# dbry/audio-resampler

Hardware: AMD Instinct MI355X
Metric: Msamples/s (out) 44.1k->48k preset -4, 8ch float32 (higher is better)
Workload: dtype i8 x 4 digits (32-bit fixed point of the f32 samples and the fp64-blended filter rows, exact i32 accumulation, one float rounding per output)

## Files before the change

audio_resampler_amd/csrc/fir_matrix_i8.hip:

```cpp
#include "fir_matrix_stream.hip.h"
#include <atomic>
#include <cstdlib>

#if !ART_WIDE

namespace {

typedef int i32x4 __attribute__ ((ext_vector_type (4)));
typedef int i32x16 __attribute__ ((ext_vector_type (16)));

constexpr int I8_KC = 32;
constexpr int I8_PITCH = 48;
constexpr int I8_COLS = 128;
constexpr int I8_MAX_PPW = 64;
constexpr int i8_ppw (int cols, int cg) { return cols / cg > I8_MAX_PPW ? I8_MAX_PPW : cols / cg; }
constexpr float I8_SCALE = 1073741824.0f;
constexpr float I8_LIMIT = 1.98f;

struct I8Geom {
    int tr;
    int cols;
    int tiles;
    int ktot;
    int g;
// ... 425 lines not shown

        for (int ch = 0; ch < nchunks; ++ch, ++qn) {
            const unsigned char *Ab = &As_ [0] [0] [0] + (qn & 1) * (int) sizeof (As_ [0]) + aoff;
            const unsigned char *Bb = &Bs_ [0] [0] [0] + (qn & 1) * (int) sizeof (Bs_ [0]) + boff;
            i32x4 av [4], bv [4];
#pragma unroll
            for (int pn = 0; pn < 4; ++pn) {
                av [pn] = *reinterpret_cast<const i32x4 *> (Ab + pn * (32 * I8_PITCH));
                bv [pn] = *reinterpret_cast<const i32x4 *> (Bb + pn * (I8_COLS * I8_PITCH));
            }
            __builtin_amdgcn_sched_group_barrier (0x100, 8, 0);
            __syncthreads ();
#define I8_PART 4
#include "fir_i8_tile32.inc"
        }
#define I8_PART 5
#include "fir_i8_tile32.inc"
    }
}

typedef __attribute__ ((address_space (3))) void *lds_ptr_t;

template <int CG, bool PASS>
__global__ __launch_bounds__ (2 * MF_THREADS) __attribute__ ((amdgpu_waves_per_eu (4, 4)))
void fir_i8_dma_kernel (ArtFirArgs a, MfmaGeom g, I8Geom q, int wgs_per_xcd)
{
    static_assert (CG >= 4 && I8_COLS % CG == 0, "16-byte vectors of 4 channels");
    constexpr int THREADS = 2 * MF_THREADS;
    constexpr int PPW = I8_COLS / CG;
    constexpr int NBUF = 3, A_BUF = 4096, B_BUF = 16384;
    __shared__ __attribute__ ((aligned (16))) unsigned char As_ [NBUF * A_BUF];
    __shared__ __attribute__ ((aligned (16))) unsigned char Bs_ [NBUF * B_BUF];

    const int tid = threadIdx.x, lane = tid & 63, wave = tid >> 6;
    const bool loader = wave >= 4;

#define I8_PART 1
#include "fir_i8_tile32.inc"
    const int total = my_tiles * nchunks;

    if (loader) {
        constexpr int VPF = CG / 4;
        constexpr unsigned int A_STEP = 4096u, B_STEP = (I8_KC / 4) * CG * 4u;
        const int lw = wave - 4;
        const int kb = 2 * lw + (lane >> 5), colquad = lane & 31, m = colquad / VPF, cv = colquad - m * VPF;
        const unsigned int boff = (unsigned int)((m * q.gq4 + kb) * CG + cv * 4) * 4u;
        const unsigned int a_off = (unsigned int)(lw * 1024 + lane * 16);
        constexpr int NB = 1;
        const int bper [NB] = { m * q.g };
        unsigned int bdel [NB] = { 0u };
        const __attribute__ ((address_space (4))) int *tile_w0 = (const __attribute__ ((address_space (4))) int *) g.tile_w0;

#define I8_PART 2
#include "fir_i8_tile32.inc"
        auto issue = [&] (int buf) -> bool {
            if (!f_live) return false;
            const unsigned int sa = (unsigned int) f_chunk * A_STEP, sb = min ((unsigned int) f_chunk * B_STEP, fb_bytes);
            const __amdgpu_buffer_rsrc_t ra_ = make_rsrc (fa_base + sa, fa_bytes - sa), rb_ = make_rsrc (fb_base + sb, fb_bytes - sb);
            __builtin_amdgcn_raw_ptr_buffer_load_lds (ra_, (lds_ptr_t)(As_ + buf * A_BUF + lw * 1024), 16, (int) a_off, 0, 0, 0);
#pragma unroll
            for (int pn = 0; pn < 4; ++pn)
                __builtin_amdgcn_raw_ptr_buffer_load_lds (rb_, (lds_ptr_t)(Bs_ + buf * B_BUF + pn * 4096 + lw * 1024), 16, (int)(boff + bdel [0]), (int)((unsigned int) pn * q.eb_plane_bytes), 0, 0);
            if (++f_chunk == nchunks) { f_chunk = 0; open_tile (); }
            return true;
        };

        open_tile ();
        bool all = true;
#pragma unroll
        for (int b = 0; b < NBUF - 1; ++b) all = issue (b) && all;
        if (all) { if constexpr (NBUF == 3) asm volatile ("s_waitcnt vmcnt(5)" ::: "memory"); else asm volatile ("s_waitcnt vmcnt(10)" ::: "memory"); }
        else asm volatile ("s_waitcnt vmcnt(0)" ::: "memory");
        __builtin_amdgcn_s_barrier ();
        int fill = NBUF - 1;
        for (int c = 0; c < total; ++c) {
            const bool more = issue (fill);
            fill = fill == NBUF - 1 ? 0 : fill + 1;
            if (more) { if constexpr (NBUF == 3) asm volatile ("s_waitcnt vmcnt(5)" ::: "memory"); else asm volatile ("s_waitcnt vmcnt(10)" ::: "memory"); }
            else asm volatile ("s_waitcnt vmcnt(0)" ::: "memory");
            __builtin_amdgcn_s_barrier ();
        }
        return;
    }

    {
        const unsigned int hw_id = __builtin_amdgcn_s_getreg ((4 - 1) << 11 | 16 << 6 | 4);
        if (hw_id & 1u) __builtin_amdgcn_s_setprio (3); else __builtin_amdgcn_s_setprio (0);
    }
    const int col = wave * 32 + (lane & 31);
    constexpr bool col_live = true;
    const int jl = col / CG, c = col - jl * CG;
    const unsigned char *Ab0 = As_ + (lane & 31) * 16 + (lane >> 5) * 512;
    const unsigned char *Bb0 = Bs_ + (lane >> 5) * 2048 + col * 4;
    const unsigned int out_off = (unsigned int)((jl * q.g * g.P + 4 * (lane >> 5)) * CG + c) * 4u;

    __builtin_amdgcn_s_barrier ();
    asm volatile ("" ::: "memory");
    int qb = 0;
    for (int within = rank; within < tiles_per_xcd; within += wgs_per_xcd) {
        int st, j0;
        if (!tile_at (within, st, j0)) continue;
#define I8_PART 3
#include "fir_i8_tile32.inc"

        for (int ch = 0; ch < nchunks; ++ch) {
            const unsigned char *Ab = Ab0 + qb * A_BUF, *Bb = Bb0 + qb * B_BUF;
            qb = qb == NBUF - 1 ? 0 : qb + 1;
            i32x4 av [4], bv [4];
#pragma unroll
            for (int pn = 0; pn < 4; ++pn) {
                av [pn] = *reinterpret_cast<const i32x4 *> (Ab + pn * 1024);
#pragma unroll
                for (int i = 0; i < 4; ++i) bv [pn] [i] = *reinterpret_cast<const int *> (Bb + pn * 4096 + i * 512);
            }
            __builtin_amdgcn_sched_group_barrier (0x100, 12, 0);
            asm volatile ("s_waitcnt lgkmcnt(0)" ::: "memory");
            __builtin_amdgcn_s_barrier ();
            asm volatile ("" ::: "memory");
#define I8_PART 4
#include "fir_i8_tile32.inc"
        }
#define I8_PART 5
#include "fir_i8_tile32.inc"
    }
}


constexpr int SL_COLS = 256, SL_THREADS = 512;
constexpr int SL_A_IMG = 8192, SL_B_IMG = 32768, SL_IMG = SL_A_IMG + SL_B_IMG, SL_BUF = 2 * SL_IMG;
constexpr int SL_WGS = 32;
constexpr int SL_MAX_SK = 64;
constexpr size_t SL_PART_BYTES = (size_t) 8 * 16 * 64 * 16;

struct I8Slab {
    int wgs_per_xcd;
    int live [8];
    unsigned char *parts;
    unsigned int *arrivals;
};


template <int CG, bool PASS>
__global__ __launch_bounds__ (SL_THREADS) __attribute__ ((amdgpu_waves_per_eu (2, 2)))
void fir_i8_slab_kernel (ArtFirArgs a, MfmaGeom g, I8Geom q, I8Slab sl)
{
    static_assert (CG >= 4 && SL_COLS % CG == 0 && SL_COLS / CG <= I8_MAX_PPW, "16-byte vectors of 4 channels");
    constexpr int THREADS = SL_THREADS;
    constexpr int PPW = SL_COLS / CG;
    __shared__ __attribute__ ((aligned (16))) unsigned char smem_ [2 * SL_BUF];

    const int tid = threadIdx.x, lane = tid & 63;
    const int wave = __builtin_amdgcn_readfirstlane (tid >> 6);

    if (a.roll_dst) {
        for (int e = (int) blockIdx.x * THREADS + tid; e < a.H * a.C; e += (int) gridDim.x * THREADS)
            matrix_roll (a.roll_dst, a.hist, a.in, a.in_frames, a.H, a.C, a.roll_appended, e);
    }
    const int W = sl.wgs_per_xcd;
    if (*q.flag == q.epoch) {
        constexpr int MF_PPW = MF_COLS / CG > MF_MAX_PPW ? MF_MAX_PPW : MF_COLS / CG;
        (void) MF_PPW;
        stand_by_tiles<CG, PASS> (a, g, W, *reinterpret_cast<float (*) [2] [32 * MF_LD]> (&smem_ [0]), *reinterpret_cast<float (*) [2] [MF_COLS * MF_LD]> (&smem_ [SL_BUF]));
        return;
    }

    const int xcd = blockIdx.x & 7, rank = blockIdx.x >> 3;
    const int nsub = q.ktot / I8_KC, nch = (nsub + 1) >> 1;
    const int L = sl.live [xcd];
    if (L <= 0) return;
    int D, S;
    {
        const int R = L / W, rem = L - R * W;
        D = rem ? (R > 0 ? R - 1 : 0) : R;
        S = L - D * W;
    }
    const int Ct = S * nch, Weff = S ? (W < Ct ? W : Ct) : 1;
    const int lo = S && rank < Weff ? (rank * Ct) / Weff : 0, hi = S && rank < Weff ? ((rank + 1) * Ct) / Weff : 0;
    const int t_first = lo / nch, t_last = hi > lo ? (hi - 1) / nch : t_first - 1;
    const int nseg = D + (t_last - t_first + 1);
    if (nseg == 0) return;
    auto segment = [&] (int k, int &within, int &c0, int &c1) {
        if (k < D) { within = rank + k * W; c0 = 0; c1 = nch; }
        else {
            const int t = t_first + (k - D);
            within = D * W + t;
            c0 = lo - t * nch; if (c0 < 0) c0 = 0;
            c1 = hi - t * nch; if (c1 > nch) c1 = nch;
        }
    };
    const int g_mask = q.g - 1, g_log2 = q.g >> 1;
    auto tile_of = [&] (int within, int &st, int &j0) {
        st = within % q.tiles;
        const int t2 = within / q.tiles, jr = t2 & g_mask, sg = xcd * q.sg_per_xcd + (t2 >> g_log2);
        j0 = ((sg * PPW) << g_log2) + jr;
    };

    constexpr int VPF = CG / 4;
    constexpr unsigned int A_STEP = 8192u, B_STEP = (I8_KC / 4) * CG * 4u;
    const int kb = 2 * (wave & 3) + (lane >> 5), colquad = (wave >> 2) * 32 + (lane & 31), m = colquad / VPF, cv = colquad - m * VPF;
    const unsigned int boff = (unsigned int)((m * q.gq4 + kb) * CG + cv * 4) * 4u;
    const unsigned int a_off = (unsigned int)(wave * 1024 + lane * 16);
    const unsigned int x_total = 4u * q.eb_plane_bytes;
    const unsigned int eb_hop = x_total - (unsigned int) q.eb_step * (unsigned int)(CG * 4);
    const int plane_step = __builtin_amdgcn_readfirstlane ((int) q.eb_plane_bytes);
    const __attribute__ ((address_space (4))) int *tile_w0 = (const __attribute__ ((address_space (4))) int *) g.tile_w0;

    int f_seg = -1, f_ch = 0, f_c1 = 0;
    unsigned long long f_live [2] = { 0ull, 0ull };
    __amdgpu_buffer_rsrc_t f_ra = make_rsrc (nullptr, 0u), f_rb = f_ra;
    unsigned int f_va = 0u, f_vb = 0u;
    auto open_segment = [&] () {
        int within, st, j0, c0;
        ++f_seg;
        segment (f_seg, within, c0, f_c1);
        tile_of (within, st, j0);
        const int la = max (tile_w0 [3 * (2 * st)] + g.w_shift + j0 * g.Q + g.head_pad, 0);
        const int eb = j0 / q.eb_periods;
        unsigned int skip = (unsigned int) max ((la >> 2) - q.b0 - eb * q.eb_step, 0) * (unsigned int)(CG * 4);
        if (skip > q.eb_plane_bytes) skip = q.eb_plane_bytes;
        const size_t from = (size_t) eb * x_total + skip;
        f_rb = make_rsrc (q.x_planes + from, (unsigned int) min (q.x_bytes - from, (size_t) 0xfffffff0u));
        const unsigned int fa_bytes = (unsigned int) nsub * A_STEP;
        f_ra = make_rsrc (q.a_planes + (size_t)(st * q.g + ((j0 + q.jr_rot) & g_mask)) * fa_bytes, fa_bytes);
        {
            const __attribute__ ((address_space (4))) unsigned long long *tm = (const __attribute__ ((address_space (4))) unsigned long long *) q.tile_masks + (st * q.g + ((j0 + q.jr_rot) & g_mask)) * 2;
            f_live [0] = tm [0] | tm [1];
            f_live [1] = tm [q.tiles * q.g * 2] | tm [q.tiles * q.g * 2 + 1];
        }
        f_ch = c0;
        f_va = a_off + (unsigned int)(2 * c0) * A_STEP;
        f_vb = boff + (unsigned int)((j0 + m * q.g) / q.eb_periods - eb) * eb_hop + (unsigned int)(2 * c0) * B_STEP;
    };
    int total = D * nch + (hi - lo), issued = 0;
    unsigned int d_va = 0u, d_vb = 0u;
    int d_skip [2] = { 0, 0 };
    int d_skip3 [2] = { 0, 0 };
    auto next_chunk = [&] () {
        if (issued < total) {
            if (f_seg < 0 || f_ch == f_c1) open_segment ();
            d_va = f_va; d_vb = f_vb;
#pragma unroll
            for (int im = 0; im < 2; ++im) {
                d_skip [im] = (wave >> 1) < 2 && !((f_live [wave >> 1] >> (2 * f_ch + im)) & 1ull) ? 0x7ffffff0 : 0;
                d_skip3 [im] = !(((f_live [0] | f_live [1]) >> (2 * f_ch + im)) & 1ull) ? 0x7ffffff0 : 0;
            }
            f_va += 2 * A_STEP; f_vb += 2 * B_STEP;
            ++f_ch; ++issued;
        }
        else { f_ra = make_rsrc (nullptr, 0u); f_rb = f_ra; }
    };
    auto piece = [&] (int buf, int idx) {
        const int im = idx / 5, pc = idx % 5;
        unsigned char *img = smem_ + buf * SL_BUF + im * SL_IMG;
        if (pc == 0) __builtin_amdgcn_raw_ptr_buffer_load_lds (f_ra, (lds_ptr_t)(img + wave * 1024), 16, (int)(d_va + (unsigned int) im * A_STEP), d_skip [im], 0, 0);
        else __builtin_amdgcn_raw_ptr_buffer_load_lds (f_rb, (lds_ptr_t)(img + SL_A_IMG + (pc - 1) * 8192 + wave * 1024), 16, (int)(d_vb + (unsigned int) im * B_STEP), pc == 4 ? (d_skip3 [im] ? d_skip3 [im] : 3 * plane_step) : (pc - 1) * plane_step, 0, 0);
    };

    if (wave & 4) __builtin_amdgcn_s_setprio (2); else __builtin_amdgcn_s_setprio (0);
    const int col = wave * 32 + (lane & 31);
    const int jl = col / CG, c = col - jl * CG;
    const unsigned char *Ab0 = smem_ + (lane >> 5) * 1024 + (lane & 31) * 16;
    const unsigned char *Bb0 = smem_ + SL_A_IMG + (wave >> 2) * 4096 + (lane >> 5) * 2048 + (col & 127) * 4;

    next_chunk ();
#pragma unroll
    for (int idx = 0; idx < 10; ++idx) piece (0, idx);
    asm volatile ("s_waitcnt vmcnt(0)" ::: "memory");
    __builtin_amdgcn_s_barrier ();
    asm volatile ("" ::: "memory");
    next_chunk ();
#pragma unroll
    for (int idx = 0; idx < 5; ++idx) piece (1, idx);
    int cur = 0;

    for (int k = 0; k < nseg; ++k) {
        int within, c0, c1, st, j0;
        segment (k, within, c0, c1);
        tile_of (within, st, j0);
        i32x16 acc [2] [5];
#pragma unroll
        for (int h = 0; h < 2; ++h)
#pragma unroll
            for (int s = 0; s < 5; ++s)
#pragma unroll
                for (int r = 0; r < 16; ++r) acc [h] [s] [r] = 0;
        unsigned long long top [2], sec [2];
        {
            const __attribute__ ((address_space (4))) unsigned long long *tm = (const __attribute__ ((address_space (4))) unsigned long long *) q.tile_masks + (st * q.g + ((j0 + q.jr_rot) & g_mask)) * 2;
            top [0] = tm [0]; top [1] = tm [1];
            sec [0] = tm [q.tiles * q.g * 2]; sec [1] = tm [q.tiles * q.g * 2 + 1];
        }
        int shift_v = q.shifts [((j0 + jl * q.g) / q.eb_periods) * CG + c];

        i32x4 av [2] [4], bv [4];
        auto read_image = [&] (int im, int sub) {
            const unsigned char *Ab = Ab0 + cur * SL_BUF + im * SL_IMG, *Bb = Bb0 + cur * SL_BUF + im * SL_IMG;
            const bool l0 = ((top [0] | top [1]) >> sub) & 1ull, l1 = ((sec [0] | sec [1]) >> sub) & 1ull;
            if (l0 | l1) {
                av [0] [1] = *reinterpret_cast<const i32x4 *> (Ab + 2048);
                av [1] [1] = *reinterpret_cast<const i32x4 *> (Ab + 2048 + 512);
#pragma unroll
                for (int i = 0; i < 4; ++i) bv [3] [i] = *reinterpret_cast<const int *> (Bb + 3 * 8192 + i * 512);
                if (l0) {
                    av [0] [0] = *reinterpret_cast<const i32x4 *> (Ab);
                    av [1] [0] = *reinterpret_cast<const i32x4 *> (Ab + 512);
                }
            }
#pragma unroll
            for (int pn = 2; pn < 4; ++pn) {
                av [0] [pn] = *reinterpret_cast<const i32x4 *> (Ab + pn * 2048);
                av [1] [pn] = *reinterpret_cast<const i32x4 *> (Ab + pn * 2048 + 512);
            }
#pragma unroll
            for (int pn = 0; pn < 3; ++pn)
#pragma unroll
                for (int i = 0; i < 4; ++i) bv [pn] [i] = *reinterpret_cast<const int *> (Bb + pn * 8192 + i * 512);
        };
        auto products = [&] (int sub, int to, int first) {
#pragma unroll
            for (int h = 0; h < 2; ++h) {
                int n = 0;
#pragma unroll
                for (int i = 2; i < 4; ++i)
#pragma unroll
                    for (int j = 0; j < 4; ++j)
                        if (i + j <= 4) {
                            acc [h] [i + j] = __builtin_amdgcn_mfma_i32_32x32x32_i8 (av [h] [i], bv [j], acc [h] [i + j], 0, 0, 0);
                            ++n;
                            if (h == 0 && n == 2) piece (to, first);
                            if (h == 0 && n == 4) piece (to, first + 1);
                            if (h == 1 && n == 1) piece (to, first + 2);
                            if (h == 1 && n == 3) piece (to, first + 3);
                            if (h == 1 && n == 5) piece (to, first + 4);
                        }
                if (h == 0) {
                    __builtin_amdgcn_sched_group_barrier (0x008, 2, 0); __builtin_amdgcn_sched_group_barrier (0x020, 1, 0);
                    __builtin_amdgcn_sched_group_barrier (0x008, 2, 0); __builtin_amdgcn_sched_group_barrier (0x020, 1, 0);
                    __builtin_amdgcn_sched_group_barrier (0x008, 1, 0);
                }
                else {
                    __builtin_amdgcn_sched_group_barrier (0x008, 1, 0); __builtin_amdgcn_sched_group_barrier (0x020, 1, 0);
                    __builtin_amdgcn_sched_group_barrier (0x008, 2, 0); __builtin_amdgcn_sched_group_barrier (0x020, 1, 0);
                    __builtin_amdgcn_sched_group_barrier (0x008, 2, 0); __builtin_amdgcn_sched_group_barrier (0x020, 1, 0);
                }
                if ((sec [h] >> sub) & 1ull) {
#pragma unroll
                    for (int j = 0; j < 4; ++j) acc [h] [1 + j] = __builtin_amdgcn_mfma_i32_32x32x32_i8 (av [h] [1], bv [j], acc [h] [1 + j], 0, 0, 0);
                }
                if ((top [h] >> sub) & 1ull) {
#pragma unroll
                    for (int j = 0; j < 4; ++j) acc [h] [j] = __builtin_amdgcn_mfma_i32_32x32x32_i8 (av [h] [0], bv [j], acc [h] [j], 0, 0, 0);
                }
            }
        };

        for (int ch = c0; ch < c1; ++ch) {
            read_image (0, 2 * ch);
            __builtin_amdgcn_sched_group_barrier (0x100, 16, 0);
            products (2 * ch, cur ^ 1, 5);
            const bool two = 2 * ch + 1 < nsub;
            if (two) read_image (1, 2 * ch + 1);
            asm volatile ("s_waitcnt lgkmcnt(0)" ::: "memory");
            asm volatile ("s_waitcnt vmcnt(0)" ::: "memory");
            if (ch == c0) asm volatile ("" : "+v" (shift_v));
            __builtin_amdgcn_s_barrier ();
            asm volatile ("" ::: "memory");
            next_chunk ();
            if (two) products (2 * ch + 1, cur, 0);
            else {
#pragma unroll
                for (int idx = 0; idx < 5; ++idx) piece (cur, idx);
            }
            asm volatile ("" ::: "memory");
            cur ^= 1;
        }

        long long tot [2] [16];
#pragma unroll
        for (int h = 0; h < 2; ++h)
#pragma unroll
            for (int r = 0; r < 16; ++r) tot [h] [r] = i8_total (acc [h] [0] [r], acc [h] [1] [r], acc [h] [2] [r], acc [h] [3] [r], acc [h] [4] [r]);
        if (c0 != 0 || c1 != nch) {
            constexpr int COHERENT = 1 | 16;
            const int t = within - D * W;
            auto owner_of = [&] (int chunk) {
                int r = (int)(((long long) chunk * Weff) / Ct);
                while (r + 1 < Weff && ((r + 1) * Ct) / Weff <= chunk) ++r;
                return r;
            };
            const int r_first = owner_of (t * nch), r_last = owner_of ((t + 1) * nch - 1);
            const unsigned int wave_bytes = 16u * 64u * 16u;
            unsigned int *count = sl.arrivals + ((size_t)(xcd * SL_MAX_SK + t) * 8 + wave);
            unsigned int before = 0u;
            bool look = k == nseg - 1 && k != D;
            if (look) {
                if (lane == 0) before = __hip_atomic_load (count, __ATOMIC_RELAXED, __HIP_MEMORY_SCOPE_AGENT);
                before = (unsigned int) __builtin_amdgcn_readfirstlane ((int) before);
                look = before == (unsigned int)(r_last - r_first);
            }
            if (!look) {
                const int which = k == D ? 0 : 1;
                const __amdgpu_buffer_rsrc_t rs_part = make_rsrc (sl.parts + ((size_t)((xcd * W + rank) * 2 + which) * 8 + wave) * wave_bytes, wave_bytes);
#pragma unroll
                for (int r = 0; r < 16; ++r) {
                    u32x4 v;
                    const unsigned long long x0 = (unsigned long long) tot [0] [r], x1 = (unsigned long long) tot [1] [r];
                    v.x = (unsigned int) x0; v.y = (unsigned int)(x0 >> 32); v.z = (unsigned int) x1; v.w = (unsigned int)(x1 >> 32);
                    __builtin_amdgcn_raw_buffer_store_b128 (v, rs_part, (r * 64 + lane) * 16, 0, COHERENT);
                }
                asm volatile ("s_waitcnt vmcnt(0)" ::: "memory");
                if (lane == 0) before = __hip_atomic_fetch_add (count, 1u, __ATOMIC_RELAXED, __HIP_MEMORY_SCOPE_AGENT);
                before = (unsigned int) __builtin_amdgcn_readfirstlane ((int) before);
            }
            if (before != (unsigned int)(r_last - r_first)) continue;
            if (lane == 0) __hip_atomic_store (count, 0u, __ATOMIC_RELAXED, __HIP_MEMORY_SCOPE_AGENT);
            for (int rr = r_first; rr <= r_last; ++rr) {
                if (rr == rank) continue;
                const int which = (rr * Ct) / Weff / nch == t ? 0 : 1;
                const __amdgpu_buffer_rsrc_t rs_part = make_rsrc (sl.parts + ((size_t)((xcd * W + rr) * 2 + which) * 8 + wave) * wave_bytes, wave_bytes);
                u32x4 v [16];
#pragma unroll
                for (int r = 0; r < 16; ++r) v [r] = __builtin_amdgcn_raw_buffer_load_b128 (rs_part, (r * 64 + lane) * 16, 0, COHERENT);
#pragma unroll
                for (int r = 0; r < 16; ++r) {
                    tot [0] [r] += (long long)((unsigned long long) v [r].x | (unsigned long long) v [r].y << 32);
                    tot [1] [r] += (long long)((unsigned long long) v [r].z | (unsigned long long) v [r].w << 32);
                }
            }
        }
        const int out_exp = -14 - shift_v;
        const unsigned int n_tile = a.n_begin + (unsigned int) j0 * g.P + (unsigned int)(st * 64);
        const int rows_valid = min (64, g.P - st * 64);
        const size_t left = (size_t)(a.n_end - n_tile) * CG * 4;
        const __amdgpu_buffer_rsrc_t rs_out = make_rsrc (a.out + (size_t) n_tile * CG, left > 0xffffff00ull ? 0xffffff00u : (unsigned int) left);
        float y [2] [16];
#pragma unroll
        for (int h = 0; h < 2; ++h) {
            const unsigned int pass_rows = PASS && 2 * st + h < g.slot_tiles ? (unsigned int) tile_w0 [3 * (2 * st + h) + 1] : 0u;
#pragma unroll
            for (int r = 0; r < 16; ++r) {
                y [h] [r] = i8_round (tot [h] [r], out_exp);
                if constexpr (PASS) {
                    const int i = h * 32 + (r & 3) + 8 * (r >> 2) + 4 * (lane >> 5);
                    if ((pass_rows >> (i & 31)) & 1u)
                        y [h] [r] = load_frame (a, INT_MIN, g.canon_ip [st * 64 + i] + g.w_shift + g.canon_fi [st * 64 + i] / a.F + (j0 + jl * q.g) * g.Q, c);
                }
            }
        }
        {
            int lane_e = lane;
            asm volatile ("" : "+v" (lane_e));
            const int qm = lane_e & 3;
            const int lo = a.n_skip != 0 && j0 == 0 && wave == 0 ? a.n_skip - st * 64 : 0;
            const int col_e = wave * 32 + (lane_e & 31), jl_e = col_e / CG, c_e = col_e - jl_e * CG;
            const unsigned int q_off = (unsigned int)((((jl_e << g_log2) * g.P) + 4 * (lane_e >> 5) + qm) * CG + (c_e & ~3)) * 4u;
#pragma unroll
            for (int h = 0; h < 2; ++h)
#pragma unroll
                for (int rb = 0; rb < 4; ++rb) {
                    unsigned int t [4];
#pragma unroll
                    for (int u = 0; u < 4; ++u) t [u] = __float_as_uint (y [h] [4 * rb + u]);
#pragma unroll
                    for (int pr = 0; pr < 4; pr += 2) {
                        const unsigned int send = (qm & 1) ? t [pr] : t [pr + 1];
                        const unsigned int recv = (unsigned int) __builtin_amdgcn_mov_dpp ((int) send, 0xB1, 0xf, 0xf, true);
                        if (qm & 1) t [pr] = recv; else t [pr + 1] = recv;
                    }
#pragma unroll
                    for (int pr = 0; pr < 2; ++pr) {
                        const unsigned int send = (qm & 2) ? t [pr] : t [pr + 2];
                        const unsigned int recv = (unsigned int) __builtin_amdgcn_mov_dpp ((int) send, 0x4E, 0xf, 0xf, true);
                        if (qm & 2) t [pr] = recv; else t [pr + 2] = recv;
                    }
                    u32x4 v; v.x = t [0]; v.y = t [1]; v.z = t [2]; v.w = t [3];
                    const int i_const = h * 32 + 8 * rb;
                    const int i = i_const + 4 * (lane >> 5) + qm;
                    const unsigned int off = i < rows_valid && (i >= lo || (lane & 31) >= CG) ? q_off + (unsigned int)(i_const * CG) * 4u : 0xfffffff0u;
                    __builtin_amdgcn_raw_buffer_store_b128 (v, rs_out, (int) off, 0, 0);
                }
        }
    }
    asm volatile ("s_waitcnt vmcnt(0)" ::: "memory");
}


}

bool artfir_i8_slab_enabled ()
{
    static const bool on = [] { const char *e = getenv ("ARTAMD_I8_SLAB"); return !(e && *e == '0'); } ();
    return on;
}
static int i8_slab_min_tiles ()
{
    static const int v = [] { const char *e = getenv ("ARTAMD_I8_SLAB_MIN"); return e && *e ? atoi (e) : 24; } ();
    return v;
}

static size_t i8_layout (const ArtFirArgs *a, const MfmaGeom &g, int cgt, I8Geom &q, char *base, unsigned int outputs = 0)
{
    if (!cgt || g.tile_rows != 32 || (g.ktot % I8_KC)) return 0;
    const unsigned int total = outputs ? outputs + (unsigned int) g.P : a->n_end - a->n_begin, periods = (total + g.P - 1) / g.P;
    q.g = (g.Q % 4 == 0) ? 1 : (g.Q % 2 == 0) ? 2 : 4;
    q.tr = 32; q.cols = I8_COLS; q.rows_cached = 0; q.jr_rot = 0; q.rows_table = 0; q.tb_base = 0.0; q.tb_lin = q.tb_w = 0; q.tb_n0 = 0u;
    if (artfir_i8_slab_enabled () && cgt >= 4) {
        const int ppw64 = i8_ppw (SL_COLS, cgt);
        const int sgs = (int)((periods + (unsigned int)(q.g * ppw64) - 1) / (unsigned int)(q.g * ppw64));
        const int per_xcd = ((sgs + 7) / 8) * q.g * ((g.P + 63) / 64);
        if (per_xcd >= i8_slab_min_tiles ()) { q.tr = 64; q.cols = SL_COLS; }
    }
    for (;;) {
        const int shift_max = (int)((q.tr - 1.0) * g.Q / g.P) + 2;
        q.ktot = ((a->T + shift_max + 3 + I8_KC - 1) / I8_KC) * I8_KC;
        if (q.tr == 64 && (q.ktot / I8_KC < 4 || q.ktot / I8_KC > 64)) { q.tr = 32; q.cols = I8_COLS; continue; }
        break;
    }
    q.tiles = (g.P + q.tr - 1) / q.tr;
    const int ppw = i8_ppw (q.cols, cgt);
    q.gq4 = q.g * g.Q / 4;
    q.super_groups = (int)((periods + (unsigned int)(q.g * ppw) - 1) / (unsigned int)(q.g * ppw));
    q.sg_per_xcd = (q.super_groups + 7) / 8;
    if (q.ktot / I8_KC > 64) return 0;
    {
        const int unit = 16 * q.g * g.Q;
        const int k = (9408 + unit / 2) / unit;
        q.eb_periods = 16 * q.g * (k > 1 ? k : 1);
    }
    q.eb_step = q.eb_periods * g.Q / 4;
    const int over_blocks = (g.Q + 2 + q.ktot + 3 + 3) / 4 + 2;
    q.eb_blocks = q.eb_step + over_blocks;
    q.ebs = (int)((periods + (unsigned int) q.eb_periods - 1) / (unsigned int) q.eb_periods);
    q.cgrp = a->C < 8 ? a->C : 8;
    q.slice_blocks = I8_STAGE_K * I8_STAGE_THREADS / q.cgrp;
    q.slices = (q.eb_blocks + q.slice_blocks - 1) / q.slice_blocks;
    q.eb_plane_bytes = (unsigned int) q.eb_blocks * (unsigned int) a->C * 4u;
    q.x_bytes = (size_t) q.ebs * 4 * q.eb_plane_bytes;
    q.b0 = 0;
    const size_t a_bytes = (size_t) q.tiles * q.g * (q.ktot / I8_KC) * (size_t)(q.tr * 128);
    const size_t masks = 2 * ((size_t) q.tiles * q.g * q.tr * 8 + (size_t) q.tiles * q.g * (q.tr / 32) * 8), shifts = (size_t) q.ebs * a->C * 4;
    const size_t teams = (size_t) q.ebs * q.slices * a->C * 4;
    const size_t head = (ART_I8_HEAD_BYTES + masks + teams + shifts + 255) & ~(size_t) 255;
    q.flag = (int *) base; q.epoch = 0;
    q.a_masks = (unsigned long long *)(base + ART_I8_HEAD_BYTES);
    q.mask_words = q.tiles * q.g * q.tr;
    q.tile_masks = q.a_masks + 2 * (size_t) q.mask_words;
    q.peaks = (unsigned int *)(base + ART_I8_HEAD_BYTES + masks);
    q.shifts = (int *)(base + ART_I8_HEAD_BYTES + masks + teams);
    q.a_planes = (unsigned char *) base + head;
    q.x_planes_w = (unsigned int *)(base + head + a_bytes); q.x_planes = (const unsigned char *) q.x_planes_w;
    q.parts = q.tr == 64 ? (unsigned char *) base + ((head + a_bytes + q.x_bytes + 255) & ~(size_t) 255) : nullptr;
    return q.tr == 64 ? ((head + a_bytes + q.x_bytes + 255) & ~(size_t) 255) + (size_t) 8 * SL_WGS * 2 * SL_PART_BYTES : head + a_bytes + q.x_bytes;
}

size_t artfir_i8_bytes (const ArtFirArgs *a, const MfmaGeom &g, int cgt, unsigned int outputs)
{
    I8Geom q;
    return i8_layout (a, g, cgt, q, nullptr, outputs ? outputs : 1u);
}

namespace {

struct RowsSetPtrs {
    unsigned long long *a_masks, *tile_masks; unsigned char *a_planes;
    float *eff; double *canon_frac; int *canon_ip, *canon_fi, *tile_w0;
};
static size_t rows_set_layout (const MfmaGeom &g, const I8Geom &q, char *base, RowsSetPtrs *out)
{
    size_t off = 0;
    auto take = [&] (size_t bytes) { const size_t at = off; off = (off + bytes + 255) & ~(size_t) 255; return at; };
    const size_t rows32 = (size_t) g.slot_tiles * 32;
    const size_t o_masks = take (2 * (size_t) q.tiles * q.g * q.tr * 8), o_tm = take (2 * (size_t) q.tiles * q.g * (q.tr / 32) * 8);
    const size_t o_planes = take ((size_t) q.tiles * q.g * (q.ktot / I8_KC) * (size_t)(q.tr * 128));
    const size_t o_eff = take (rows32 * g.ktot * sizeof (float)), o_frac = take (rows32 * sizeof (double));
    const size_t o_ip = take (rows32 * sizeof (int)), o_fi = take (rows32 * sizeof (int)), o_w0 = take ((size_t) 3 * g.slot_tiles * sizeof (int));
    if (out && base) {
        out->a_masks = (unsigned long long *)(base + o_masks); out->tile_masks = (unsigned long long *)(base + o_tm); out->a_planes = (unsigned char *)(base + o_planes);
        out->eff = (float *)(base + o_eff); out->canon_frac = (double *)(base + o_frac); out->canon_ip = (int *)(base + o_ip); out->canon_fi = (int *)(base + o_fi);
        out->tile_w0 = (int *)(base + o_w0);
    }
    return off;
}

}

extern "C" {
size_t arthip_fir_rows_cache_bytes (void) { return sizeof (ArtRowsCache); }
void arthip_fir_rows_cache_reset (void *cache)
{
    ArtRowsCache *rc = (ArtRowsCache *) cache;
    if (rc) { for (int k = 0; k < 4; ++k) rc->valid [k] = 0; rc->f_valid = 0; }
}
void arthip_fir_rows_cache_free (void *cache)
{
    ArtRowsCache *rc = (ArtRowsCache *) cache;
    if (rc) {
        free (rc->c_ph); free (rc->c_ip); free (rc->c_fi); rc->c_ph = nullptr; rc->c_ip = rc->c_fi = nullptr; rc->cap = 0; rc->canon_valid = 0;
    }
}
}

size_t artfir_i8_rows_bytes (const ArtFirArgs *a, const MfmaGeom &g, int cgt, unsigned int outputs)
{
    I8Geom q;
    if (!i8_layout (a, g, cgt, q, nullptr, outputs ? outputs : 1u)) return 0;
    return (size_t)(4 / q.g) * (rows_set_layout (g, q, nullptr, nullptr) + 4096);
}

namespace {

typedef void (*I8TileKernel) (ArtFirArgs, MfmaGeom, I8Geom, int);
typedef void (*I8SlabKernel) (ArtFirArgs, MfmaGeom, I8Geom, I8Slab);
#define I8_PICK(KERNEL, CGT) (pass ? KERNEL<CGT, true> : KERNEL<CGT, false>)
I8TileKernel i8_tile_kernel (int cgt, bool pass)
{
    switch (cgt) {
        case 32: return I8_PICK (fir_i8_dma_kernel, 32);
        case 16: return I8_PICK (fir_i8_dma_kernel, 16);
        case 8: return I8_PICK (fir_i8_dma_kernel, 8);
        case 4: return I8_PICK (fir_i8_dma_kernel, 4);
        case 2: return I8_PICK (fir_i8_stream_kernel, 2);
        default: return I8_PICK (fir_i8_stream_kernel, 1);
    }
}
I8SlabKernel i8_slab_kernel (int cgt, bool pass)
{
    switch (cgt) {
        case 32: return I8_PICK (fir_i8_slab_kernel, 32);
        case 16: return I8_PICK (fir_i8_slab_kernel, 16);
        case 8: return I8_PICK (fir_i8_slab_kernel, 8);
        default: return I8_PICK (fir_i8_slab_kernel, 4);
    }
}
#undef I8_PICK
// ... 130 lines not shown
```

Before: 84050.

## Prefetch first chunk before roll and defer split-tile fixup to overlap waiting

Result: no change. 83220 (-1.0%).

```diff
diff --git a/audio_resampler_amd/csrc/fir_matrix_i8.hip b/audio_resampler_amd/csrc/fir_matrix_i8.hip
--- a/audio_resampler_amd/csrc/fir_matrix_i8.hip
+++ b/audio_resampler_amd/csrc/fir_matrix_i8.hip
@@ -601,22 +601,10 @@
     const int tid = threadIdx.x, lane = tid & 63;
     const int wave = __builtin_amdgcn_readfirstlane (tid >> 6);
 
-    if (a.roll_dst) {
-        for (int e = (int) blockIdx.x * THREADS + tid; e < a.H * a.C; e += (int) gridDim.x * THREADS)
-            matrix_roll (a.roll_dst, a.hist, a.in, a.in_frames, a.H, a.C, a.roll_appended, e);
-    }
     const int W = sl.wgs_per_xcd;
-    if (*q.flag == q.epoch) {
-        constexpr int MF_PPW = MF_COLS / CG > MF_MAX_PPW ? MF_MAX_PPW : MF_COLS / CG;
-        (void) MF_PPW;
-        stand_by_tiles<CG, PASS> (a, g, W, *reinterpret_cast<float (*) [2] [32 * MF_LD]> (&smem_ [0]), *reinterpret_cast<float (*) [2] [MF_COLS * MF_LD]> (&smem_ [SL_BUF]));
-        return;
-    }
-
     const int xcd = blockIdx.x & 7, rank = blockIdx.x >> 3;
     const int nsub = q.ktot / I8_KC, nch = (nsub + 1) >> 1;
-    const int L = sl.live [xcd];
-    if (L <= 0) return;
+    const int L = sl.live [xcd] > 0 ? sl.live [xcd] : 0;
     int D, S;
     {
         const int R = L / W, rem = L - R * W;
@@ -627,7 +615,6 @@
     const int lo = S && rank < Weff ? (rank * Ct) / Weff : 0, hi = S && rank < Weff ? ((rank + 1) * Ct) / Weff : 0;
     const int t_first = lo / nch, t_last = hi > lo ? (hi - 1) / nch : t_first - 1;
     const int nseg = D + (t_last - t_first + 1);
-    if (nseg == 0) return;
     auto segment = [&] (int k, int &within, int &c0, int &c1) {
         if (k < D) { within = rank + k * W; c0 = 0; c1 = nch; }
         else {
@@ -705,15 +692,31 @@
         else __builtin_amdgcn_raw_ptr_buffer_load_lds (f_rb, (lds_ptr_t)(img + SL_A_IMG + (pc - 1) * 8192 + wave * 1024), 16, (int)(d_vb + (unsigned int) im * B_STEP), pc == 4 ? (d_skip3 [im] ? d_skip3 [im] : 3 * plane_step) : (pc - 1) * plane_step, 0, 0);
     };
 
+    if (nseg != 0) {
+        next_chunk ();
+#pragma unroll
+        for (int idx = 0; idx < 10; ++idx) piece (0, idx);
+    }
+    if (a.roll_dst) {
+        for (int e = (int) blockIdx.x * THREADS + tid; e < a.H * a.C; e += (int) gridDim.x * THREADS)
+            matrix_roll (a.roll_dst, a.hist, a.in, a.in_frames, a.H, a.C, a.roll_appended, e);
+    }
+    if (*q.flag == q.epoch) {
+        constexpr int MF_PPW = MF_COLS / CG > MF_MAX_PPW ? MF_MAX_PPW : MF_COLS / CG;
+        (void) MF_PPW;
+        asm volatile ("s_waitcnt vmcnt(0)" ::: "memory");
+        __syncthreads ();
+        stand_by_tiles<CG, PASS> (a, g, W, *reinterpret_cast<float (*) [2] [32 * MF_LD]> (&smem_ [0]), *reinterpret_cast<float (*) [2] [MF_COLS * MF_LD]> (&smem_ [SL_BUF]));
+        return;
+    }
+    if (nseg == 0) return;
+
     if (wave & 4) __builtin_amdgcn_s_setprio (2); else __builtin_amdgcn_s_setprio (0);
     const int col = wave * 32 + (lane & 31);
     const int jl = col / CG, c = col - jl * CG;
     const unsigned char *Ab0 = smem_ + (lane >> 5) * 1024 + (lane & 31) * 16;
     const unsigned char *Bb0 = smem_ + SL_A_IMG + (wave >> 2) * 4096 + (lane >> 5) * 2048 + (col & 127) * 4;
 
-    next_chunk ();
-#pragma unroll
-    for (int idx = 0; idx < 10; ++idx) piece (0, idx);
     asm volatile ("s_waitcnt vmcnt(0)" ::: "memory");
     __builtin_amdgcn_s_barrier ();
     asm volatile ("" ::: "memory");
@@ -721,6 +724,87 @@
 #pragma unroll
     for (int idx = 0; idx < 5; ++idx) piece (1, idx);
     int cur = 0;
+
+    constexpr int COHERENT = 1 | 16;
+    const unsigned int wave_bytes = 16u * 64u * 16u;
+    auto owner_of = [&] (int chunk) {
+        int r = (int)(((long long) chunk * Weff) / Ct);
+        while (r + 1 < Weff && ((r + 1) * Ct) / Weff <= chunk) ++r;
+        return r;
+    };
+    auto arrivals_of = [&] (int t) { return sl.arrivals + ((size_t)(xcd * SL_MAX_SK + t) * 8 + wave); };
+    auto add_parts = [&] (int t, int r_first, int r_last, int but, long long (&tot) [2] [16]) {
+        for (int rr = r_first; rr <= r_last; ++rr) {
+            if (rr == but) continue;
+            const int which = (rr * Ct) / Weff / nch == t ? 0 : 1;
+            const __amdgpu_buffer_rsrc_t rs_part = make_rsrc (sl.parts + ((size_t)((xcd * W + rr) * 2 + which) * 8 + wave) * wave_bytes, wave_bytes);
+            u32x4 v [16];
+#pragma unroll
+            for (int r = 0; r < 16; ++r) v [r] = __builtin_amdgcn_raw_buffer_load_b128 (rs_part, (r * 64 + lane) * 16, 0, COHERENT);
+#pragma unroll
+            for (int r = 0; r < 16; ++r) {
+                tot [0] [r] += (long long)((unsigned long long) v [r].x | (unsigned long long) v [r].y << 32);
+                tot [1] [r] += (long long)((unsigned long long) v [r].z | (unsigned long long) v [r].w << 32);
+            }
+        }
+    };
+    int defer = -1;
+    bool owe = false;
+    int shift_v = 0;
+    auto finish = [&] (int st, int j0, long long (&tot) [2] [16]) {
+            const int out_exp = -14 - shift_v;
+            const unsigned int n_tile = a.n_begin + (unsigned int) j0 * g.P + (unsigned int)(st * 64);
+            const int rows_valid = min (64, g.P - st * 64);
+            const size_t left = (size_t)(a.n_end - n_tile) * CG * 4;
+            const __amdgpu_buffer_rsrc_t rs_out = make_rsrc (a.out + (size_t) n_tile * CG, left > 0xffffff00ull ? 0xffffff00u : (unsigned int) left);
+            float y [2] [16];
+#pragma unroll
+            for (int h = 0; h < 2; ++h) {
+                const unsigned int pass_rows = PASS && 2 * st + h < g.slot_tiles ? (unsigned int) tile_w0 [3 * (2 * st + h) + 1] : 0u;
+#pragma unroll
+                for (int r = 0; r < 16; ++r) {
+                    y [h] [r] = i8_round (tot [h] [r], out_exp);
+                    if constexpr (PASS) {
+                        const int i = h * 32 + (r & 3) + 8 * (r >> 2) + 4 * (lane >> 5);
+                        if ((pass_rows >> (i & 31)) & 1u)
+                            y [h] [r] = load_frame (a, INT_MIN, g.canon_ip [st * 64 + i] + g.w_shift + g.canon_fi [st * 64 + i] / a.F + (j0 + jl * q.g) * g.Q, c);
+                    }
+                }
+            }
+            {
+                int lane_e = lane;
+                asm volatile ("" : "+v" (lane_e));
+                const int qm = lane_e & 3;
+                const int lo = a.n_skip != 0 && j0 == 0 && wave == 0 ? a.n_skip - st * 64 : 0;
+                const int col_e = wave * 32 + (lane_e & 31), jl_e = col_e / CG, c_e = col_e - jl_e * CG;
+                const unsigned int q_off = (unsigned int)((((jl_e << g_log2) * g.P) + 4 * (lane_e >> 5) + qm) * CG + (c_e & ~3)) * 4u;
+#pragma unroll
+                for (int h = 0; h < 2; ++h)
+#pragma unroll
+                    for (int rb = 0; rb < 4; ++rb) {
+                        unsigned int t [4];
+#pragma unroll
+                        for (int u = 0; u < 4; ++u) t [u] = __float_as_uint (y [h] [4 * rb + u]);
+#pragma unroll
+                        for (int pr = 0; pr < 4; pr += 2) {
+                            const unsigned int send = (qm & 1) ? t [pr] : t [pr + 1];
+                            const unsigned int recv = (unsigned int) __builtin_amdgcn_mov_dpp ((int) send, 0xB1, 0xf, 0xf, true);
+                            if (qm & 1) t [pr] = recv; else t [pr + 1] = recv;
+                        }
+#pragma unroll
+                        for (int pr = 0; pr < 2; ++pr) {
+                            const unsigned int send = (qm & 2) ? t [pr] : t [pr + 2];
+                            const unsigned int recv = (unsigned int) __builtin_amdgcn_mov_dpp ((int) send, 0x4E, 0xf, 0xf, true);
+                            if (qm & 2) t [pr] = recv; else t [pr + 2] = recv;
+                        }
+                        u32x4 v; v.x = t [0]; v.y = t [1]; v.z = t [2]; v.w = t [3];
+                        const int i_const = h * 32 + 8 * rb;
+                        const int i = i_const + 4 * (lane_e >> 5) + qm;
+                        const unsigned int off = i < rows_valid && (i >= lo || (lane_e & 31) >= CG) ? q_off + (unsigned int)(i_const * CG) * 4u : 0xfffffff0u;
+                        __builtin_amdgcn_raw_buffer_store_b128 (v, rs_out, (int) off, 0, 0);
+                    }
+            }
+    };
 
     for (int k = 0; k < nseg; ++k) {
         int within, c0, c1, st, j0;
@@ -739,7 +823,7 @@
             top [0] = tm [0]; top [1] = tm [1];
             sec [0] = tm [q.tiles * q.g * 2]; sec [1] = tm [q.tiles * q.g * 2 + 1];
         }
-        int shift_v = q.shifts [((j0 + jl * q.g) / q.eb_periods) * CG + c];
+        shift_v = q.shifts [((j0 + jl * q.g) / q.eb_periods) * CG + c];
 
         i32x4 av [2] [4], bv [4];
         auto read_image = [&] (int im, int sub) {
@@ -814,7 +898,16 @@
             if (ch == c0) asm volatile ("" : "+v" (shift_v));
             __builtin_amdgcn_s_barrier ();
             asm volatile ("" ::: "memory");
+            unsigned int arrived = 0u;
+            if (ch == c0 && defer >= 0) {
+                if (lane == 0) arrived = __hip_atomic_fetch_add (arrivals_of (t_first), 1u, __ATOMIC_RELAXED, __HIP_MEMORY_SCOPE_AGENT);
+            }
             next_chunk ();
+            if (ch == c0 && defer >= 0) {
+                owe = (unsigned int) __builtin_amdgcn_readfirstlane ((int) arrived) == (unsigned int) defer;
+                if (owe && lane == 0) __hip_atomic_store (arrivals_of (t_first), 0u, __ATOMIC_RELAXED, __HIP_MEMORY_SCOPE_AGENT);
+                defer = -1;
+            }
             if (two) products (2 * ch + 1, cur, 0);
             else {
 #pragma unroll
@@ -830,16 +923,9 @@
 #pragma unroll
             for (int r = 0; r < 16; ++r) tot [h] [r] = i8_total (acc [h] [0] [r], acc [h] [1] [r], acc [h] [2] [r], acc [h] [3] [r], acc [h] [4] [r]);
         if (c0 != 0 || c1 != nch) {
-            constexpr int COHERENT = 1 | 16;
             const int t = within - D * W;
-            auto owner_of = [&] (int chunk) {
-                int r = (int)(((long long) chunk * Weff) / Ct);
-                while (r + 1 < Weff && ((r + 1) * Ct) / Weff <= chunk) ++r;
-                return r;
-            };
             const int r_first = owner_of (t * nch), r_last = owner_of ((t + 1) * nch - 1);
-            const unsigned int wave_bytes = 16u * 64u * 16u;
-            unsigned int *count = sl.arrivals + ((size_t)(xcd * SL_MAX_SK + t) * 8 + wave);
+            unsigned int *count = arrivals_of (t);
             unsigned int before = 0u;
             bool look = k == nseg - 1 && k != D;
             if (look) {
@@ -857,78 +943,29 @@
                     v.x = (unsigned int) x0; v.y = (unsigned int)(x0 >> 32); v.z = (unsigned int) x1; v.w = (unsigned int)(x1 >> 32);
                     __builtin_amdgcn_raw_buffer_store_b128 (v, rs_part, (r * 64 + lane) * 16, 0, COHERENT);
                 }
+                if (k == D && k + 1 < nseg) { defer = r_last - r_first; continue; }
                 asm volatile ("s_waitcnt vmcnt(0)" ::: "memory");
                 if (lane == 0) before = __hip_atomic_fetch_add (count, 1u, __ATOMIC_RELAXED, __HIP_MEMORY_SCOPE_AGENT);
                 before = (unsigned int) __builtin_amdgcn_readfirstlane ((int) before);
             }
             if (before != (unsigned int)(r_last - r_first)) continue;
             if (lane == 0) __hip_atomic_store (count, 0u, __ATOMIC_RELAXED, __HIP_MEMORY_SCOPE_AGENT);
-            for (int rr = r_first; rr <= r_last; ++rr) {
-                if (rr == rank) continue;
-                const int which = (rr * Ct) / Weff / nch == t ? 0 : 1;
-                const __amdgpu_buffer_rsrc_t rs_part = make_rsrc (sl.parts + ((size_t)((xcd * W + rr) * 2 + which) * 8 + wave) * wave_bytes, wave_bytes);
-                u32x4 v [16];
-#pragma unroll
-                for (int r = 0; r < 16; ++r) v [r] = __builtin_amdgcn_raw_buffer_load_b128 (rs_part, (r * 64 + lane) * 16, 0, COHERENT);
-#pragma unroll
-                for (int r = 0; r < 16; ++r) {
-                    tot [0] [r] += (long long)((unsigned long long) v [r].x | (unsigned long long) v [r].y << 32);
-                    tot [1] [r] += (long long)((unsigned long long) v [r].z | (unsigned long long) v [r].w << 32);
-                }
-            }
-        }
-        const int out_exp = -14 - shift_v;
-        const unsigned int n_tile = a.n_begin + (unsigned int) j0 * g.P + (unsigned int)(st * 64);
-        const int rows_valid = min (64, g.P - st * 64);
-        const size_t left = (size_t)(a.n_end - n_tile) * CG * 4;
-        const __amdgpu_buffer_rsrc_t rs_out = make_rsrc (a.out + (size_t) n_tile * CG, left > 0xffffff00ull ? 0xffffff00u : (unsigned int) left);
-        float y [2] [16];
-#pragma unroll
-        for (int h = 0; h < 2; ++h) {
-            const unsigned int pass_rows = PASS && 2 * st + h < g.slot_tiles ? (unsigned int) tile_w0 [3 * (2 * st + h) + 1] : 0u;
-#pragma unroll
-            for (int r = 0; r < 16; ++r) {
-                y [h] [r] = i8_round (tot [h] [r], out_exp);
-                if constexpr (PASS) {
-                    const int i = h * 32 + (r & 3) + 8 * (r >> 2) + 4 * (lane >> 5);
-                    if ((pass_rows >> (i & 31)) & 1u)
-                        y [h] [r] = load_frame (a, INT_MIN, g.canon_ip [st * 64 + i] + g.w_shift + g.canon_fi [st * 64 + i] / a.F + (j0 + jl * q.g) * g.Q, c);
-                }
-            }
-        }
-        {
-            int lane_e = lane;
-            asm volatile ("" : "+v" (lane_e));
-            const int qm = lane_e & 3;
-            const int lo = a.n_skip != 0 && j0 == 0 && wave == 0 ? a.n_skip - st * 64 : 0;
-            const int col_e = wave * 32 + (lane_e & 31), jl_e = col_e / CG, c_e = col_e - jl_e * CG;
-            const unsigned int q_off = (unsigned int)((((jl_e << g_log2) * g.P) + 4 * (lane_e >> 5) + qm) * CG + (c_e & ~3)) * 4u;
-#pragma unroll
-            for (int h = 0; h < 2; ++h)
-#pragma unroll
-                for (int rb = 0; rb < 4; ++rb) {
-                    unsigned int t [4];
-#pragma unroll
-                    for (int u = 0; u < 4; ++u) t [u] = __float_as_uint (y [h] [4 * rb + u]);
-#pragma unroll
-                    for (int pr = 0; pr < 4; pr += 2) {
-                        const unsigned int send = (qm & 1) ? t [pr] : t [pr + 1];
-                        const unsigned int recv = (unsigned int) __builtin_amdgcn_mov_dpp ((int) send, 0xB1, 0xf, 0xf, true);
-                        if (qm & 1) t [pr] = recv; else t [pr + 1] = recv;
-                    }
-#pragma unroll
-                    for (int pr = 0; pr < 2; ++pr) {
-                        const unsigned int send = (qm & 2) ? t [pr] : t [pr + 2];
-                        const unsigned int recv = (unsigned int) __builtin_amdgcn_mov_dpp ((int) send, 0x4E, 0xf, 0xf, true);
-                        if (qm & 2) t [pr] = recv; else t [pr + 2] = recv;
-                    }
-                    u32x4 v; v.x = t [0]; v.y = t [1]; v.z = t [2]; v.w = t [3];
-                    const int i_const = h * 32 + 8 * rb;
-                    const int i = i_const + 4 * (lane >> 5) + qm;
-                    const unsigned int off = i < rows_valid && (i >= lo || (lane & 31) >= CG) ? q_off + (unsigned int)(i_const * CG) * 4u : 0xfffffff0u;
-                    __builtin_amdgcn_raw_buffer_store_b128 (v, rs_out, (int) off, 0, 0);
-                }
-        }
+            add_parts (t, r_first, r_last, rank, tot);
+        }
+        finish (st, j0, tot);
+    }
+    if (owe) {
+        int within, c0, c1, st, j0;
+        segment (D, within, c0, c1);
+        tile_of (within, st, j0);
+        shift_v = q.shifts [((j0 + jl * q.g) / q.eb_periods) * CG + c];
+        long long tot [2] [16];
+#pragma unroll
+        for (int h = 0; h < 2; ++h)
+#pragma unroll
+            for (int r = 0; r < 16; ++r) tot [h] [r] = 0;
+        add_parts (t_first, owner_of (t_first * nch), owner_of ((t_first + 1) * nch - 1), -1, tot);
+        finish (st, j0, tot);
     }
     asm volatile ("s_waitcnt vmcnt(0)" ::: "memory");
 }
```
